# Harvard-AI-and-Robotics-Lab/FairFedMed

Measured on AMD Instinct MI355X. Metric: images/sec per client-round, ViT-B/16 FairLoRA r=8, bs=32 224^2, higher is better.
Workload: dtype bf16; 1 GPU; configs[1]: 1-client ViT-B/16 FairLoRA rank=8 G=3, bs=32 synthetic 224x224x3, fwd+bwd+SGD per step; global_batch=32, clients=1, trainable_elems=741952, loss_finite=1, launch=replay, rccl_ranks=1

## Files before the change

fairfedmed_amd/_lib.py:

```python
from __future__ import annotations

import ctypes as C
import os
from typing import Optional

import torch

_HERE = os.path.dirname(os.path.abspath(__file__))
LIB_PATH = os.environ.get("FFM_LIB_PATH") or os.path.join(_HERE, "csrc", "libffm_hip.so")

F32, BF16, F32_X3, F16 = 0, 1, 2, 3
F32_X3_W16 = 4
EPI_BIAS, EPI_LORA, EPI_LORA_KR, EPI_RESIDUAL, EPI_GELU, EPI_DGELU, EPI_RANKOP = 1, 2, 4, 8, 16, 32, 64
EPI_ROWSTATS, EPI_LNIN, EPI_LGRAD, EPI_BNBWD = 128, 256, 512, 1024
EPI_LNB_STAT, EPI_LNB_APPLY = 2048, 4096
EPI_GELU_ONLY = 8192
ABI_VERSION = 14

_vp, _i32, _i64, _f32 = C.c_void_p, C.c_int32, C.c_int64, C.c_float


class GemmArgs(C.Structure):
    _fields_ = [
        ("a", _vp), ("b", _vp), ("c", _vp),
# ... 64 lines not shown
    "ffm_bn_bwd": [_vp, _vp, _vp, _vp, _vp, _vp, _vp, _i32, _vp, _vp, _vp, _vp, _vp, _i32, _i32, _i32, _vp],
    "ffm_avgpool2": [_vp, _vp, _i32, _i32, _i32, _i32, _i32, _i32, _vp],
    "ffm_add": [_vp, _vp, _vp, C.c_int64, _i32, _vp],
    "ffm_relu_bwd": [_vp, _vp, _vp, C.c_int64, _i32, _vp],
    "ffm_attnpool_tokens": [_vp, _vp, _vp, _i32, _i32, _i32, _i32, _i32, _vp],
    "ffm_conv3x3_nhwc": [_vp, _vp, _vp, _i32, _i32, _i32, _i32, _i32, _i32, _vp, _vp, _i64, _vp, _i32, _vp],
    "ffm_conv3x3_nhwc_bnbwd": [_vp, _vp, _vp, _i32, _i32, _i32, _i32, _i32, _i32, _vp, _vp, _i64, _vp, _vp, _vp, _vp, _vp, _i32, _vp],
    "ffm_conv3x3_colstat_rows": [_i32, _i32, _i32, _i32, _i32, _i32, _i64, _i32],
    "ffm_eval_counts": [_vp, _vp, _vp, _i32, _i32, _vp, _vp],
    "ffm_eval_counts_ws_bytes": [_i32],
    "ffm_eval_counts_sorted": [_vp, _vp, _vp, _i32, _i32, _vp, _vp, _i64, _vp],
    "ffm_ot_head_fwd": [_vp] * 10 + [_i32] * 6 + [_f32, _f32, _i32, _f32, _i32, _vp],
    "ffm_ot_head_bwd": [_vp] * 8 + [_i32] * 6 + [_vp],
    "ffm_expand_u8": [_vp, _vp, _i32, _i32, _i32, _i32, _vp],
    "ffm_resize_u8": [_vp, _vp, _vp, _vp, _vp, _i32, _i32, _i32, _i32, _i32, _vp],
    "ffm_scale_check": [_vp, _f32, _i64, _vp, _vp],
    "ffm_attention_fwd": [_vp, _vp, _vp, _i32, _i32, _i32, _i32, _i32, _vp],
    "ffm_attention_bwd": [_vp, _vp, _vp, _vp, _vp, _vp, _i32, _i32, _i32, _i32, _i32, _vp],
    "ffm_attention_bwd_lnstat_ok": [_i32, _i32, _i32],
    "ffm_attention_bwd_lnstat": [_vp, _vp, _vp, _vp, _vp, _vp, _vp, _vp, _vp, _i32, _i32, _i32, _i32, _i32, _vp],
    "ffm_lora_down": [_vp, _i32, _vp, _i32, _vp, _vp, _i32, _i32, _i32, _i32, _i32, _f32, _f32, _vp, _vp, _vp, _vp,
                      _i32, _vp],
    "ffm_lora_down_blocks": [_i32, _i32, _i32, _i32],
    "ffm_lora_down_blocks_max": [_i32, _i32, _i32, _i32],
    "ffm_lora_grad_partial": [_vp, _i32, _vp, _i32, _i32, _i32, _vp, _i32, _vp],
    "ffm_lora_grad_partial_ln": [_vp, _i32, _vp, _vp, _vp, _vp, _vp, _i32, _i32, _i32, _vp, _i32, _vp],
    "ffm_lora_grad_splits": [_i32],
    "ffm_reduce_partials": [_vp, _i32, _i32, _vp, _i32, _i32, _i32, _vp],
    "ffm_reduce_partials_multi": [_vp, _i32, _i32, _vp],
    "ffm_head_fwd": [_vp, _vp, _vp, _vp, _vp, _vp, _i32, _i32, _i32, _i32, _i32, _vp],
    "ffm_ce_loss": [_vp, _vp, _vp, _vp, _vp, _vp, _vp, _i32, _i32, _i32, _vp],
    "ffm_ce_fair_loss": [_vp] * 10 + [_i32, _i32, _i32, _i32, _f32, _i32, _vp],
    "ffm_head_bwd": [_vp, _vp, _vp, _vp, _vp, _vp, _vp, _vp, _i32, _i32, _i32, _i32, _i32, _vp],
    "ffm_text_embed": [_vp, _vp, _vp, _i32, _vp, _vp, _i32, _i32, _i32, _i32, _i32, _vp],
    "ffm_text_tail_fwd": [_vp] * 10 + [_i32] * 4 + [_vp],
    "ffm_text_tail_bwd": [_vp] * 11 + [_i32] * 5 + [_vp],
    "ffm_text_ctx_grad": [_vp, _vp, _i32, _i32, _i32, _i32, _i32, _vp],
    "ffm_sgd_momentum": [_vp, _vp, _vp, _i64, _f32, _f32, _f32, _i32, _vp],
    "ffm_sgd_momentum_n": [_vp, _vp, _vp, _i64, _f32, _f32, _f32, _i32, _i32, _vp],
    "ffm_sgd_momentum_dev": [_vp, _vp, _vp, _i64, _vp, _i32, _vp, _vp],
    "ffm_loss_scale": [_vp, _i64, _vp, _vp],
    "ffm_unscale_check": [_vp, _i64, _vp, _vp],
    "ffm_sgd_momentum_gated": [_vp, _vp, _vp, _i64, _f32, _f32, _f32, _i32, _i32, _vp, _vp],
    "ffm_optim_state_rows": [_i32],
    "ffm_optim_step": [_vp, _vp, _vp, _i64, _i32, _vp, _i32, _vp, _vp],
    "ffm_optim_step_dev": [_vp, _vp, _vp, _i64, _i32, _vp, _i32, _vp, _vp],
    "ffm_scale_by": [_vp, _vp, _vp, _i64, _vp],
    "ffm_scale_acc": [_vp, _vp, _vp, _i64, _vp],
    "ffm_fedavg_finish": [_vp, _vp, _vp, _i64, _vp, _i32, _i32, _i32, _i32, _f32, _vp],
    "ffm_cast_f32_to": [_vp, _vp, _i64, _i32, _vp],
    "ffm_cast_to_f32": [_vp, _vp, _i64, _i32, _vp],
    "ffm_transpose_cast": [_vp, _vp, _i32, _i32, _i32, _vp],
}

_lib: Optional[C.CDLL] = None


def load() -> C.CDLL:
    global _lib
    if _lib is not None:
        return _lib
    if not os.path.exists(LIB_PATH):
        raise RuntimeError(
            f"{LIB_PATH} is missing: build it with `python -m fairfedmed_amd.build` "
            "(the FairLoRA engine has no fallback path)")
    lib = C.CDLL(LIB_PATH)
# ... 39 lines not shown
```

fairfedmed_amd/csrc/head.hip:

```cpp
#include "common.h"

namespace {

constexpr int HD_MAXV = 4;
constexpr int HD_MAXC = 8;

constexpr int HD_NW = 16;

template <typename T>
__global__ __launch_bounds__(64 * HD_NW) void head_fwd_kernel(const T* __restrict__ f, const float* __restrict__ tbar,
                                                       const float* __restrict__ logit_scale,
                                                       float* __restrict__ fbar, float* __restrict__ rnorm,
                                                       float* __restrict__ logits, int L, int D, int n_cls) {
    __shared__ float red[HD_NW / 2][4 * 64 * HD_MAXV];
    const int b = blockIdx.x, lane = threadIdx.x & 63, wave = threadIdx.x >> 6;
    const int nchunk = D >> 2;
    f32x4 acc[HD_MAXV];
#pragma unroll
    for (int i = 0; i < HD_MAXV; ++i) acc[i] = (f32x4){0.f, 0.f, 0.f, 0.f};
    for (int l = 1 + wave; l < L; l += HD_NW) {
        const T* fr = f + ((size_t)b * L + l) * D;
        f32x4 v[HD_MAXV];
        float ss = 0.f;
#pragma unroll
// ... 25 lines not shown
#pragma unroll
                for (int e = 0; e < 4; ++e) red[wave - HD_NW / 2][c * 4 + e] = acc[i][e];
            }
        }
    }
    __syncthreads();
    if (wave < HD_NW / 2) {
#pragma unroll
        for (int i = 0; i < HD_MAXV; ++i) {
            const int c = lane + 64 * i;
            if (c < nchunk) {
#pragma unroll
                for (int e = 0; e < 4; ++e) red[wave][c * 4 + e] += acc[i][e];
            }
        }
    }
    __syncthreads();
    const float inv = 1.0f / (float)(L - 1);
    for (int d = threadIdx.x; d < D; d += 64 * HD_NW) {
        float s = 0.f;
#pragma unroll
        for (int w = 0; w < HD_NW / 2; ++w) s += red[w][d];
        s *= inv;
        red[0][d] = s;
        fbar[(size_t)b * D + d] = s;
    }
    __syncthreads();
    const float scale = expf(logit_scale[0]);
    for (int c = wave; c < n_cls; c += HD_NW) {
        float s = 0.f;
        for (int d = lane; d < D; d += 64) s += red[0][d] * tbar[(size_t)c * D + d];
        s = wave_sum(s);
        if (lane == 0) logits[(size_t)b * n_cls + c] = scale * s;
    }
}

__global__ __launch_bounds__(256) void ce_loss_kernel(const float* __restrict__ logits_img,
                                                      const int64_t* __restrict__ label, float* __restrict__ logits,
                                                      float* __restrict__ prob, float* __restrict__ loss,
                                                      float* __restrict__ dlogits_img, int32_t* __restrict__ finite,
                                                      int nb, int S, int n_cls) {
    __shared__ float part[256];
    float my = 0.f;
    for (int b = threadIdx.x; b < nb; b += 256) {
        float lg[HD_MAXC];
        float mx = -INFINITY;
        for (int c = 0; c < n_cls; ++c) {
            float s = 0.f;
            for (int k = 0; k < S; ++k) s += logits_img[((size_t)b * S + k) * n_cls + c];
            lg[c] = s / (float)S;
            logits[(size_t)b * n_cls + c] = lg[c];
            mx = fmaxf(mx, lg[c]);
        }
        float se = 0.f;
        for (int c = 0; c < n_cls; ++c) se += expf(lg[c] - mx);
        const float lse = mx + logf(se);
        const int y = (int)label[b];
        my += lse - lg[y];
        for (int c = 0; c < n_cls; ++c) {
            const float pc = expf(lg[c] - lse);
            prob[(size_t)b * n_cls + c] = pc;
            const float dl = (pc - (c == y ? 1.f : 0.f)) / (float)nb / (float)S;
            for (int k = 0; k < S; ++k) dlogits_img[((size_t)b * S + k) * n_cls + c] = dl;
        }
    }
    part[threadIdx.x] = my;
// ... 152 lines not shown
            for (int i = 0; i < HD_MAXV; ++i) {
                const int c = lane + 64 * i;
                if (c < nchunk) Vec4<T>::store(dr + c * 4, (f32x4){0.f, 0.f, 0.f, 0.f});
            }
            continue;
        }
        const T* fr = f + ((size_t)b * L + l) * D;
        const float rn = rnorm[(size_t)b * L + l];
        f32x4 y[HD_MAXV];
        float dot = 0.f;
#pragma unroll
        for (int i = 0; i < HD_MAXV; ++i) {
            const int c = lane + 64 * i;
            if (c < nchunk) {
                const f32x4 v = Vec4<T>::load(fr + c * 4);
#pragma unroll
                for (int e = 0; e < 4; ++e) { y[i][e] = v[e] * rn; dot += y[i][e] * dyb[c * 4 + e]; }
            }
        }
        dot = wave_sum(dot);
#pragma unroll
        for (int i = 0; i < HD_MAXV; ++i) {
            const int c = lane + 64 * i;
            if (c < nchunk) {
                f32x4 o;
#pragma unroll
                for (int e = 0; e < 4; ++e) o[e] = (dyb[c * 4 + e] - y[i][e] * dot) * rn;
                Vec4<T>::store(dr + c * 4, o);
            }
        }
    }
}

__global__ __launch_bounds__(256) void head_dtbar_kernel(const float* __restrict__ fbar,
                                                         const float* __restrict__ logit_scale,
                                                         const float* __restrict__ dlogits, float* __restrict__ dtbar,
                                                         int B, int D, int n_cls) {
    const int i = blockIdx.x * blockDim.x + threadIdx.x;
    if (i >= n_cls * D) return;
    const int c = i / D, d = i % D;
    float s = 0.f;
    int b = 0;
    for (; b + 8 <= B; b += 8) {
        float dl[8], fb[8];
#pragma unroll
        for (int u = 0; u < 8; ++u) {
            dl[u] = dlogits[(size_t)(b + u) * n_cls + c];
            fb[u] = fbar[(size_t)(b + u) * D + d];
        }
#pragma unroll
        for (int u = 0; u < 8; ++u) s += dl[u] * fb[u];
    }
    for (; b < B; ++b) s += dlogits[(size_t)b * n_cls + c] * fbar[(size_t)b * D + d];
    dtbar[i] = s * expf(logit_scale[0]);
}

}

extern "C" int ffm_head_fwd(const void* f, const float* tbar, const float* logit_scale, float* fbar, float* rnorm,
                            float* logits_img, int B, int L, int D, int n_cls, int dtype, void* stream) {
    if (!f || !tbar || !logit_scale || !fbar || !rnorm || !logits_img) return FFM_EINVAL;
    if (B <= 0 || L <= 1 || D <= 0 || (D & 3) || D > 4 * 64 * HD_MAXV || n_cls <= 0 || n_cls > HD_MAXC) return FFM_EINVAL;
    hipStream_t s = (hipStream_t)stream;
    if (dtype == FFM_BF16)
        hipLaunchKernelGGL((head_fwd_kernel<bf16_t>), dim3(B), dim3(64 * HD_NW), 0, s, (const bf16_t*)f, tbar, logit_scale,
                           fbar, rnorm, logits_img, L, D, n_cls);
    else if (dtype == FFM_F32)
        hipLaunchKernelGGL((head_fwd_kernel<float>), dim3(B), dim3(64 * HD_NW), 0, s, (const float*)f, tbar, logit_scale,
                           fbar, rnorm, logits_img, L, D, n_cls);
    else
        return FFM_EINVAL;
    FFM_CHECK_LAUNCH();
    return FFM_OK;
}

extern "C" int ffm_ce_loss(const float* logits_img, const int64_t* label, float* logits, float* prob, float* loss,
                           float* dlogits_img, int32_t* finite_flag, int nb, int S, int n_cls, void* stream) {
    if (!logits_img || !label || !logits || !prob || !loss || !dlogits_img) return FFM_EINVAL;
    if (nb <= 0 || S <= 0 || n_cls <= 0 || n_cls > HD_MAXC) return FFM_EINVAL;
    hipLaunchKernelGGL(ce_loss_kernel, dim3(1), dim3(256), 0, (hipStream_t)stream, logits_img, label, logits, prob,
                       loss, dlogits_img, finite_flag, nb, S, n_cls);
    FFM_CHECK_LAUNCH();
    return FFM_OK;
}

extern "C" int ffm_ce_fair_loss(const float* logits_img, const int64_t* label, const int32_t* attr, float* logits,
                                float* prob, float* loss, float* terms, float* gstat, float* dlogits_img,
                                int32_t* finite_flag, int nb, int S, int n_cls, int G, float lambda, int with_grad,
                                void* stream) {
    if (!logits_img || !label || !attr || !logits || !prob || !loss || !terms || !dlogits_img) return FFM_EINVAL;
    if (nb <= 0 || S <= 0 || n_cls <= 0 || n_cls > HD_MAXC || G <= 0 || G > FFM_MAX_GROUPS) return FFM_EINVAL;
    hipLaunchKernelGGL(ce_fair_loss_kernel, dim3(1), dim3(256), 0, (hipStream_t)stream, logits_img, label, attr, logits,
                       prob, loss, terms, gstat, dlogits_img, finite_flag, nb, S, n_cls, G, lambda, with_grad ? 1 : 0);
    FFM_CHECK_LAUNCH();
    return FFM_OK;
}

extern "C" int ffm_head_bwd(const void* f, const float* tbar, const float* logit_scale, const float* fbar,
                            const float* rnorm, const float* dlogits_img, void* df, float* dtbar, int B, int L, int D,
                            int n_cls, int dtype, void* stream) {
    if (!f || !tbar || !logit_scale || !fbar || !rnorm || !dlogits_img || !df || !dtbar) return FFM_EINVAL;
    if (B <= 0 || L <= 1 || D <= 0 || (D & 3) || D > 4 * 64 * HD_MAXV || n_cls <= 0 || n_cls > HD_MAXC) return FFM_EINVAL;
    hipStream_t s = (hipStream_t)stream;
    if (dtype == FFM_BF16)
// ... 14 lines not shown
```

fairfedmed_amd/engine.py:

```python
from __future__ import annotations

import os
from dataclasses import dataclass
from typing import Dict, List, Optional, Tuple

import torch

from . import _lib as L
from ._lib import is16 as _is16
from . import ops
from .config import ModelCfg
from .data import NativeBatch
from .synth import manifest, trainable_keys

Tensor = torch.Tensor


def _round_up(x: int, m: int) -> int:
    return (x + m - 1) // m * m


class FlatParams:

    def __init__(self, cfg: ModelCfg, device):
# ... 370 lines not shown

    @grad_scale.setter
    def grad_scale(self, value: float) -> None:
        value = float(value)
        if not (value > 0.0) or value != value or value == float("inf"):
            raise ValueError(f"grad_scale must be a positive finite number, got {value!r}")
        if self.scale_state is None:
            if value != 1.0:
                raise ValueError("grad_scale exists in the IEEE-half mode only")
            return
        self.scale_state[:2].copy_(torch.tensor([value, 1.0 / value]))
        self.scale_state[5:6].fill_(max(value, float(self.scale_state[5])))

    def overflow_steps(self) -> int:
        return int(self.scale_state[4]) if self.scale_state is not None else 0

    def __init__(self, cfg: ModelCfg, state_dict: Dict[str, Tensor], dtype=torch.bfloat16, max_images: int = 32,
                 device: str = "cuda:0", max_infer_images: Optional[int] = None):
        if not torch.cuda.is_available():
            raise RuntimeError("FairLoRAEngine needs an MI355X GPU; there is no CPU path")
        from . import _lib
        _lib.load()
        if cfg.vision.head_dim != 64 or cfg.text.width // cfg.text.heads != 64:
            raise ValueError("attention kernels are built for head_dim 64 (all CLIP towers)")
        self.cfg, self.dtype, self.device = cfg, dtype, torch.device(device)
        self.max_images = max_images
        v, t = cfg.vision, cfg.text
        self.sw = Switches.from_env()
        self.fused_rank = 0 < cfg.lora.rank <= 16
        self.pack_plan = None
        self._pack_event = None
        self.pk_out: Dict[str, Tensor] = {}
        self.use_replay = True
        self.no_colstats, self.bn_bwd_fused = False, self.sw.bn_bwd_fused
        self.params = FlatParams(cfg, self.device)
        self.params.load(state_dict)
        self.n_text = cfg.n_prompts * cfg.n_cls
        self.txt_len = min(t.context_length, max(cfg.eot) + 1)
        assert self.txt_len >= 1 + cfg.n_ctx
        if not all(0 <= int(e) < self.txt_len for e in cfg.eot):
            raise ValueError(f"EOT positions {list(cfg.eot)} must lie inside the {self.txt_len} text rows that are kept "
                             f"(context_length {t.context_length})")
        self.txt = _Stack(t.width, t.heads, t.layers, self.txt_len, self.n_text, True, 0, torch.float32, self.device,
                          self.sw, x3=(_is16(dtype)))
        dev, f32 = self.device, torch.float32
        self._init_vision(max_images)
        self.load_frozen(state_dict)
        self._init_vision_late()
        self.feat = torch.zeros(max_images * v.tokens, v.out_dim, device=dev, dtype=dtype)
        self.dfeat = torch.zeros_like(self.feat)
        self.fbar = torch.zeros(max_images, v.out_dim, device=dev, dtype=f32)
        self.rnorm = torch.zeros(max_images * v.tokens, device=dev, dtype=f32)
        self.logits_img = torch.zeros(max_images, cfg.n_cls, device=dev, dtype=f32)
        self.dlogits_img = torch.zeros_like(self.logits_img)
        self.logits = torch.zeros(max_images, cfg.n_cls, device=dev, dtype=f32)
        self.prob = torch.zeros_like(self.logits)
        self.loss = torch.zeros(1, device=dev, dtype=f32)
        self.finite = torch.ones(1, device=dev, dtype=torch.int32)
        self.scale_state = None
        if dtype == torch.float16:
            s0 = self.sw.f16_grad_scale
            self.scale_state = torch.tensor([s0, 1.0 / s0, 1.0, 0.0, 0.0, s0, self.sw.f16_growth_interval, 1.0],
                                            device=dev, dtype=f32)
        self.dtbar = torch.zeros(cfg.n_cls, v.out_dim, device=dev, dtype=f32)
        self.attr_i32 = torch.zeros(max_images, device=dev, dtype=torch.int32)
        self.label_buf = torch.zeros(max_images, device=dev, dtype=torch.int64)
        self._counts_buf = None
        self._fair_lam, self._fair_grad, self._fair_step = 0.0, False, False
        self.loss_terms = torch.zeros(2, device=dev, dtype=f32)
        self.group_conf = torch.zeros(ops.MAX_GROUPS, 2, device=dev, dtype=f32)
        self.tbar_buf = torch.zeros(cfg.n_cls, v.out_dim, device=dev, dtype=f32)
        self.ot = cfg.ot if cfg.ot != "None" else None
        if self.ot:
            if self.ot not in ops.OT_MODES:
                raise NotImplementedError(cfg.ot)
            P, M, N = max_images * cfg.n_cls, v.tokens - 1, cfg.n_prompts
            self.dtn = torch.zeros(N * cfg.n_cls, v.out_dim, device=dev, dtype=f32)
            self.ot_sim = torch.zeros(P * M * N, device=dev, dtype=f32)
            self.ot_T = torch.zeros_like(self.ot_sim)
            self.ot_errs = torch.zeros(cfg.ot_max_iter * P, device=dev, dtype=f32)
            self.ot_istop = torch.zeros(1, device=dev, dtype=torch.int32)
            self.ot_tsum = torch.zeros(P, device=dev, dtype=f32)
            self.ot_dtn_part = torch.zeros(max_images * N * cfg.n_cls * v.out_dim, device=dev, dtype=f32)
        self.step_plans: Dict[tuple, list] = {}
# ... 502 lines not shown
        if train and self.sops.glob:
            self._glue(self.sops.prepare)
        ops.gemm_nt(ws.cols[:images * P], self.conv_w, ws.patch_out[:images * P], b_packed=self.pk_out.get("conv_w"))
        lb0 = bufs.layer(0, rows)
        ops.embed_lnpre(ws.patch_out[:images * P], self.cls, self.pos, self.lnpre[0], self.lnpre[1],
                        lb0.x, images, L, rowstat=lb0.rowp)
        if train:
            self._rank_operands_ready()
        out = self._stack_forward(self.vis, rows, images, a32, L * S, bufs)
        ops.layernorm_fwd(out, ws.hpost[:rows], self.lnpost[0], self.lnpost[1], ws.post_stats[0], ws.post_stats[1])
        ops.gemm_nt(ws.hpost[:rows], self.proj_t, ws.feat[:rows], b_packed=self.pk_out.get("proj_t"))
        if wait is not None:
            self._ev_wait(torch.cuda.current_stream(self.device), wait)
        self._head_forward(rows, images, L, ws)

    def _pack_rank_operands(self) -> None:
        if self.pack_plan is not None:
            self.pack_plan.run()

    def _rank_operands_ready(self) -> None:
        ev = self._pack_event
        if ev is None:
            self._pack_rank_operands()
        else:
            self._ev_wait(torch.cuda.current_stream(self.device), ev)

    def _head_forward(self, rows: int, images: int, L: int, ws=None) -> None:
        cfg = self.cfg
        ws = self if ws is None else ws
        if self.ot:
            ops.ot_head_fwd(ws.feat[:rows], self.tn_buf, self.logit_scale, ws.rnorm, ws.ot_sim, ws.ot_T, ws.ot_errs,
                            ws.ot_istop, ws.ot_tsum, ws.logits_img, images, L, cfg.n_cls, cfg.n_prompts, self.ot,
                            cfg.ot_eps, cfg.ot_thresh, cfg.ot_max_iter, cfg.ot_top_percent)
        else:
            ops.head_fwd(ws.feat[:rows], self.tbar_buf, self.logit_scale, ws.fbar, ws.rnorm, ws.logits_img,
                         images, L, cfg.n_cls)

    def _head_backward(self, rows: int, images: int, L: int) -> None:
        cfg = self.cfg
        if self.ot:
            P = cfg.n_prompts * cfg.n_cls
            ops.ot_head_bwd(self.feat[:rows], self.tn_buf, self.logit_scale, self.rnorm, self.ot_T, self.dlogits_img,
                            self.dfeat[:rows], self.ot_dtn_part, images, L, cfg.n_cls, cfg.n_prompts)
            ops.reduce_partials(self.ot_dtn_part, images, P * self.cfg.vision.out_dim, self.dtn.view(-1))
        else:
            ops.head_bwd(self.feat[:rows], self.tbar_buf, self.logit_scale, self.fbar, self.rnorm, self.dlogits_img,
                         self.dfeat[:rows], self.dtbar, images, L, cfg.n_cls)

    def _vision_backward(self, b: int, S: int, has_attr: bool) -> None:
        cfg, v = self.cfg, self.cfg.vision
        images, L = b * S, v.tokens
        rows = images * L
        a32 = self.attr_i32[:b] if has_attr else None
        ops.gemm_nt(self.dfeat[:rows], self.proj, self.vis.dh[:rows], b_packed=self.pk_out.get("proj"))
        gl = self.vis.rank > 0
        ops.layernorm_bwd(self.vis.dh[:rows], self.vis.x[v.layers][:rows], self.lnpost[0], self.post_stats[0],
                          self.post_stats[1], None, (self.vis.g_l[v.layers - 1] if gl else self.vis.g)[:rows])
        self._stack_backward(self.vis, rows, images, a32, L * S, self.is3d, grad_in_last=gl)
        if self.is3d:
            P = v.grid * v.grid
            ops.embed_lnpre_bwd(self.vis.g[:rows], self.patch_out[:images * P], self.pos, self.lnpre[0],
                                self.dpatch[:images * P], images, L)
            ops.gemm_nt(self.dpatch[:images * P], self.conv_w_t, self.dcols[:images * P])

    @torch.no_grad()
    def forward(self, image: Tensor, attr: Optional[Tensor] = None) -> Tensor:
        if self.sops.type != "FairLoRA":
            attr = None
        b, S = self._load_inputs(image, attr, None)
        self._text_forward(False)
        self._vision_forward(b, S, attr is not None)
        return self.logits_img[:b * S].view(b, S, -1).mean(1)

    def _infer_prepare(self) -> None:
        self._pack_rank_operands()
        if self.sops.glob:
            self.sops.prepare()
# ... 9 lines not shown
                self.prev, eng._in_session = eng._in_session, True
                return eng

            def __exit__(self, *a):
                eng._in_session = self.prev
                return False
        return _Session()

    @torch.no_grad()
    def infer(self, image: Tensor, attr: Optional[Tensor] = None) -> Tensor:
        if self.sops.type != "FairLoRA":
            attr = None
        ws = self.infer_ws
        b, S = self._load_inputs(image, attr, None, ws)
        if not self._in_session:
            self._infer_prepare()
        self._vision_forward(b, S, attr is not None, ws=ws)
        return ws.logits_img[:b * S].view(b, S, -1).mean(1)

    def _step_body(self, b: int, S: int, has_attr: bool) -> None:
        cfg, v = self.cfg, self.cfg.vision
        main = torch.cuda.current_stream(self.device)
        images, L = b * S, v.tokens
        rows = images * L
        a32 = self.attr_i32[:b] if has_attr else None
        self._ev_record(self.ev_start, main)
        self._ev_wait(self.side, self.ev_start)
        with self._on(self.side):
            self._pack_rank_operands()
            self._ev_record(self.ev_pack, self.side)
            self._text_forward(True, self.side)
        self._ev_record(self.ev_text_fwd, self.side)
        self._pack_event = self.ev_pack
        try:
            self._vision_forward(b, S, has_attr, wait=self.ev_text_fwd)
        finally:
            self._pack_event = None
        if self._fair_step:
            ops.ce_fair_loss(self.logits_img, self.label_buf, self.attr_i32, self.logits, self.prob, self.loss,
                             self.loss_terms, self.group_conf, self.dlogits_img, self.finite, b, S, cfg.n_cls,
                             self._fair_groups(), self._fair_lam, self._fair_grad)
        else:
            ops.ce_loss(self.logits_img, self.label_buf, self.logits, self.prob, self.loss, self.dlogits_img,
                        self.finite, b, S, cfg.n_cls)
        if self.scale_state is not None:
            ops.loss_scale(self.dlogits_img[:b * S], self.scale_state)
        self._head_backward(rows, images, L)
        self._ev_record(self.ev_head_bwd, main)
        self._ev_wait(self.side, self.ev_head_bwd)
        with self._on(self.side):
            if self._counts_buf is not None:
                ops.eval_counts(self.prob[:b], self.label_buf[:b], None, 0, method="pairs", out=self._counts_buf)
            self._text_backward(self.side)
        self._ev_record(self.ev_text_bwd, self.side)
        self._vision_backward(b, S, has_attr)
        self._ev_wait(main, self.ev_text_bwd)

    def forward_backward(self, image: Tensor, attr: Optional[Tensor], label: Tensor) -> Dict[str, Tensor]:
        fair = self._fair_lam != 0.0 and attr is not None
        loss_attr = attr if fair else None
        if self.sops.type != "FairLoRA":
            attr = None
        with torch.no_grad():
            b, S = self._load_inputs(image, attr if attr is not None else loss_attr, label)
            key = (b, S, attr is not None, torch.cuda.current_stream(self.device).cuda_stream) + (("fair",) if fair else ())
            self._fair_step = fair
            plan = self.step_plans.get(key) if self.use_replay else None
            if plan is not None:
                for f in plan:
                    f()
            elif self.use_replay:
                plan = []
                with ops.record(plan):
                    self._step_body(b, S, attr is not None)
                self.step_plans[key] = plan
            else:
                self._step_body(b, S, attr is not None)
            if self.is3d:
                images, P, D = b * S, self.cfg.vision.grid ** 2, self.cfg.dim_per_3d_slice
                ops.slice_bwd(self.dcols[:images * P], self._image, self.conv_out[:images], self.mnmx, self.mm_cnt,
                              self.dconv[:images], self.ab_part, self.gmm, self.wpart, D, self.cfg.vision.patch,
                              self.cfg.pixel_std)
                nw = 3 * D * 25 + 3
                off = self.params.offsets["proj_per_3d_slice.weight"][0]
                assert self.params.offsets["proj_per_3d_slice.bias"][0] == off + nw - 3
                nblk = ops.slice_wgrad_blocks(self.cfg.vision.image_size, self.cfg.vision.image_size)
                ops.reduce_partials(self.wpart, images * nblk, nw, self.params.grad[off:off + nw])
            if self.scale_state is not None:
                ops.unscale_check(self.params.grad, self.scale_state)
        out = {"loss": self.loss, "logits": self.logits[:b], "prob": self.prob[:b], "finite": self.finite}
        if self._counts_buf is not None:
            out["counts"] = self._counts_buf
        if fair:
            out["loss_terms"], out["group_conf"] = self.loss_terms, self.group_conf[:self._fair_groups()]
        return out

    @torch.no_grad()
    def sgd_step(self, lr: float, momentum: float, weight_decay: float, repeats: int = 1) -> None:
# ... 142 lines not shown
```

fairfedmed_amd/ops.py:

```python
from __future__ import annotations

import ctypes as C
from typing import Optional

import torch

from . import _lib as L

Tensor = torch.Tensor

_REC = None


class record:
    def __init__(self, plan: list):
        self.plan = plan

    def __enter__(self):
        global _REC
        self.prev, _REC = _REC, self.plan
        return self.plan

    def __exit__(self, *a):
        global _REC
# ... 698 lines not shown

def ce_loss(logits_img: Tensor, label: Tensor, logits: Tensor, prob: Tensor, loss: Tensor, dlogits_img: Tensor,
            finite: Optional[Tensor], nb: int, S: int, n_cls: int) -> None:
    _dev(logits_img, label, logits, prob, loss, dlogits_img, finite)
    assert label.dtype == torch.int64 and (finite is None or finite.dtype == torch.int32)
    _call("ffm_ce_loss", L.ptr(_f32(logits_img)), L.ptr(label), L.ptr(_f32(logits)), L.ptr(_f32(prob)),
                                 L.ptr(_f32(loss)), L.ptr(_f32(dlogits_img)), L.ptr(finite), nb, S, n_cls,
                                 L.stream_ptr())


def ce_fair_loss(logits_img: Tensor, label: Tensor, attr: Tensor, logits: Tensor, prob: Tensor, loss: Tensor,
                 terms: Tensor, gstat: Optional[Tensor], dlogits_img: Tensor, finite: Optional[Tensor], nb: int, S: int,
                 n_cls: int, G: int, lam: float, with_grad: bool = False) -> None:
    _dev(logits_img, label, attr, logits, prob, loss, terms, gstat, dlogits_img, finite)
    assert label.dtype == torch.int64 and attr.dtype == torch.int32 and (finite is None or finite.dtype == torch.int32)
    assert attr.is_contiguous() and attr.numel() >= nb and label.numel() >= nb and terms.numel() >= 2
    assert logits_img.numel() >= nb * S * n_cls and dlogits_img.numel() >= nb * S * n_cls
    assert logits.numel() >= nb * n_cls and prob.numel() >= nb * n_cls and (gstat is None or gstat.numel() >= 2 * G)
    _call("ffm_ce_fair_loss", L.ptr(_f32(logits_img)), L.ptr(label), L.ptr(attr), L.ptr(_f32(logits)), L.ptr(_f32(prob)),
          L.ptr(_f32(loss)), L.ptr(_f32(terms)), L.ptr(_f32(gstat)), L.ptr(_f32(dlogits_img)), L.ptr(finite), nb, S,
          n_cls, G, float(lam), int(bool(with_grad)), L.stream_ptr())


def head_bwd(f: Tensor, tbar: Tensor, logit_scale: Tensor, fbar: Tensor, rnorm: Tensor, dlogits_img: Tensor,
             df: Tensor, dtbar: Tensor, B: int, Ltok: int, n_cls: int) -> None:
    _dev(f, tbar, logit_scale, fbar, rnorm, dlogits_img, df, dtbar)
    D = f.shape[1]
    assert f.dtype == df.dtype and df.is_contiguous()
    _call("ffm_head_bwd", L.ptr(f), L.ptr(_f32(tbar)), L.ptr(_f32(logit_scale)), L.ptr(_f32(fbar)),
                                  L.ptr(_f32(rnorm)), L.ptr(_f32(dlogits_img)), L.ptr(df), L.ptr(_f32(dtbar)), B,
                                  Ltok, D, n_cls, L.dtype_code(f.dtype), L.stream_ptr())


def sgd_momentum(p: Tensor, g: Tensor, buf: Tensor, lr: float, momentum: float, weight_decay: float,
                 first_step: bool, repeats: int = 1) -> None:
    _dev(p, g, buf)
    if repeats == 1:
        _call("ffm_sgd_momentum", L.ptr(_f32(p)), L.ptr(_f32(g)), L.ptr(_f32(buf)), p.numel(), lr, momentum,
              weight_decay, int(first_step), L.stream_ptr())
    else:
        _call("ffm_sgd_momentum_n", L.ptr(_f32(p)), L.ptr(_f32(g)), L.ptr(_f32(buf)), p.numel(), lr, momentum,
              weight_decay, int(first_step), int(repeats), L.stream_ptr())


MAX_GROUPS = 8
SCALE_STATE = 8


def loss_scale(p: Tensor, state: Tensor) -> None:
    _dev(p, state)
    assert p.is_contiguous() and state.numel() == SCALE_STATE
    _call("ffm_loss_scale", L.ptr(_f32(p)), p.numel(), L.ptr(_f32(state)), L.stream_ptr())


def unscale_check(g: Tensor, state: Tensor) -> None:
    _dev(g, state)
    assert g.is_contiguous() and state.numel() == SCALE_STATE
    _call("ffm_unscale_check", L.ptr(_f32(g)), g.numel(), L.ptr(_f32(state)), L.stream_ptr())


def sgd_momentum_gated(p: Tensor, g: Tensor, buf: Tensor, lr: float, momentum: float, weight_decay: float,
                       first_step: bool, repeats: int, state: Tensor) -> None:
    _dev(p, g, buf, state)
    _call("ffm_sgd_momentum_gated", L.ptr(_f32(p)), L.ptr(_f32(g)), L.ptr(_f32(buf)), p.numel(), lr, momentum,
          weight_decay, int(first_step), int(repeats), L.ptr(_f32(state)), L.stream_ptr())

# ... 87 lines not shown
```

include/ffm_hip.h:

```cpp
#ifndef FFM_HIP_H
#define FFM_HIP_H

#include <stdint.h>

#ifdef __cplusplus
extern "C" {
#endif

#define FFM_F32 0
#define FFM_BF16 1
#define FFM_F32_X3 2
#define FFM_F16 3
#define FFM_F32_X3_W16 4

#define FFM_OK 0
#define FFM_EINVAL (-1)
#define FFM_EUNSUP (-2)

#define FFM_MAX_RANK 32
#define FFM_MAX_GROUPS 8

#define FFM_ABI_VERSION 14
int ffm_abi_version(void);

// ... 162 lines not shown
                          float* part, int dtype, void* stream);
int ffm_lora_grad_partial_ln(const void* x, int ldx, const float* v, const float* mean, const float* rstd,
                             const float* gamma, const float* beta, int M, int K, int r, float* part, int dtype,
                             void* stream);
int ffm_lora_grad_splits(int M);

int ffm_reduce_partials(const float* part, int nsplit, int n, float* out, int transpose_K,
                        int transpose_r, int accumulate, void* stream);

typedef struct ffm_reduce_desc {
    const float* part;
    float* out;
    int32_t nsplit, n, transpose_K, transpose_r;
} ffm_reduce_desc;
int ffm_reduce_partials_multi(const ffm_reduce_desc* descs_dev, int ndesc, int max_n, void* stream);

int ffm_head_fwd(const void* f, const float* tbar, const float* logit_scale, float* fbar,
                 float* rnorm, float* logits_img, int B, int L, int D, int n_cls, int dtype,
                 void* stream);

int ffm_ce_loss(const float* logits_img, const int64_t* label, float* logits, float* prob,
                float* loss, float* dlogits_img, int32_t* finite_flag, int nb, int S, int n_cls,
                void* stream);

int ffm_ce_fair_loss(const float* logits_img, const int64_t* label, const int32_t* attr,
                     float* logits, float* prob, float* loss, float* terms, float* gstat,
                     float* dlogits_img, int32_t* finite_flag, int nb, int S, int n_cls, int G,
                     float lambda, int with_grad, void* stream);

int ffm_head_bwd(const void* f, const float* tbar, const float* logit_scale, const float* fbar,
                 const float* rnorm, const float* dlogits_img, void* df, float* dtbar, int B,
                 int L, int D, int n_cls, int dtype, void* stream);

int ffm_text_embed(const float* prefix, const float* ctx, const float* suffix, int suffix_rows, const float* pos, float* x,
                   int n_prompts, int n_cls, int n_ctx, int TL, int w, void* stream);
int ffm_text_tail_fwd(const float* x, const int32_t* eot_row, const float* lnw, const float* lnb, const float* proj,
                      float* tf, float* tn, float* rnorm, float* stats, float* tbar, int n_prompts, int n_cls, int w,
                      int D, void* stream);
int ffm_text_tail_bwd(const float* x, const int32_t* eot_row, const float* lnw, const float* proj, const float* tn,
                      const float* rnorm, const float* stats, const float* dtbar, const float* dtn, float* dy, float* g,
                      int n_prompts, int n_cls, int TL, int w, int D, void* stream);
int ffm_text_ctx_grad(const float* g, float* dctx, int n_prompts, int n_cls, int n_ctx, int TL, int w, void* stream);

int ffm_expand_u8(const uint8_t* src, float* dst, int B, int C1, int HW, int rep, void* stream);

#define FFM_RESIZE_MAX_TAPS 32
int ffm_resize_u8(const uint8_t* pix, const int32_t* geom, const int32_t* tab_start, const float* tab_w, float* dst,
                  int B, int C1, int rep, int R, int T, void* stream);

#define FFM_EVAL_SLOTS 10
int ffm_eval_counts(const float* prob, const int64_t* label, const int64_t* attr, int N, int G, uint64_t* out,
                    void* stream);
int64_t ffm_eval_counts_ws_bytes(int N);
int ffm_eval_counts_sorted(const float* prob, const int64_t* label, const int64_t* attr, int N, int G, uint64_t* out,
                           void* workspace, int64_t workspace_bytes, void* stream);

int ffm_ot_head_fwd(const void* f, const float* tn, const float* logit_scale, float* rnorm, float* sim, float* T,
                    float* errs, int32_t* istop, float* tsum, float* logits_img, int B, int L, int D, int n_cls,
                    int N, int mode, float eps, float thresh, int max_iter, float top_percent, int dtype, void* stream);
int ffm_ot_head_bwd(const void* f, const float* tn, const float* logit_scale, const float* rnorm, const float* T,
                    const float* dlogits_img, void* df, float* dtn_part, int B, int L, int D, int n_cls, int N,
                    int dtype, void* stream);

int ffm_sgd_momentum(float* p, const float* g, float* buf, int64_t n, float lr, float momentum,
                     float weight_decay, int first_step, void* stream);

// ... 48 lines not shown
```

Before: 7203 images/sec.

## Split head forward across waves and fuse CE loss into head backward

Replaces the single-block-per-image head forward with a multi-block kernel that writes per-wave partial pooled features. A new head backward kernel reduces those partials itself, computes logits and the cross-entropy gradient inline, and spreads the dfeat writes over four blocks per image. The full CE loss and dtbar computation move to the side stream, off the main critical path. This path is limited to non-fair, S==1, non-OT, unscaled steps and adds an fpart buffer plus redundant per-block reductions.

```diff
diff --git a/fairfedmed_amd/_lib.py b/fairfedmed_amd/_lib.py
--- a/fairfedmed_amd/_lib.py
+++ b/fairfedmed_amd/_lib.py
@@ -120,6 +120,9 @@
     "ffm_ce_loss": [_vp, _vp, _vp, _vp, _vp, _vp, _vp, _i32, _i32, _i32, _vp],
     "ffm_ce_fair_loss": [_vp] * 10 + [_i32, _i32, _i32, _i32, _f32, _i32, _vp],
     "ffm_head_bwd": [_vp, _vp, _vp, _vp, _vp, _vp, _vp, _vp, _i32, _i32, _i32, _i32, _i32, _vp],
+    "ffm_head_fwd_split": [_vp, _vp, _vp, _i32, _i32, _i32, _i32, _vp],
+    "ffm_head_bwd_self": [_vp] * 10 + [_i32, _i32, _i32, _i32, _i32, _vp],
+    "ffm_head_dtbar": [_vp, _vp, _vp, _vp, _i32, _i32, _i32, _vp],
     "ffm_text_embed": [_vp, _vp, _vp, _i32, _vp, _vp, _i32, _i32, _i32, _i32, _i32, _vp],
     "ffm_text_tail_fwd": [_vp] * 10 + [_i32] * 4 + [_vp],
     "ffm_text_tail_bwd": [_vp] * 11 + [_i32] * 5 + [_vp],
diff --git a/fairfedmed_amd/csrc/head.hip b/fairfedmed_amd/csrc/head.hip
--- a/fairfedmed_amd/csrc/head.hip
+++ b/fairfedmed_amd/csrc/head.hip
@@ -81,6 +81,65 @@
         for (int d = lane; d < D; d += 64) s += red[0][d] * tbar[(size_t)c * D + d];
         s = wave_sum(s);
         if (lane == 0) logits[(size_t)b * n_cls + c] = scale * s;
+    }
+}
+
+constexpr int HD_PF = 4;
+
+__device__ __forceinline__ float sum_sq4(const f32x4 v) {
+#pragma clang fp contract(off)
+    return v[0] * v[0] + v[1] * v[1] + v[2] * v[2] + v[3] * v[3];
+}
+
+template <typename T>
+__global__ __launch_bounds__(64) void head_fwd_split_kernel(const T* __restrict__ f, float* __restrict__ fpart,
+                                                            float* __restrict__ rnorm, int L, int D) {
+    const int b = blockIdx.x, wave = blockIdx.y, lane = threadIdx.x;
+    const int nchunk = D >> 2;
+    f32x4 acc[HD_MAXV];
+#pragma unroll
+    for (int i = 0; i < HD_MAXV; ++i) acc[i] = (f32x4){0.f, 0.f, 0.f, 0.f};
+    for (int l0 = 1 + wave; l0 < L; l0 += HD_NW * HD_PF) {
+        f32x4 v[HD_PF][HD_MAXV];
+#pragma unroll
+        for (int u = 0; u < HD_PF; ++u) {
+            const int l = l0 + u * HD_NW;
+            const T* fr = f + ((size_t)b * L + (l < L ? l : l0)) * D;
+#pragma unroll
+            for (int i = 0; i < HD_MAXV; ++i) {
+                const int c = lane + 64 * i;
+                if (c < nchunk) v[u][i] = Vec4<T>::load(fr + c * 4);
+            }
+        }
+#pragma unroll
+        for (int u = 0; u < HD_PF; ++u) {
+            const int l = l0 + u * HD_NW;
+            if (l >= L) break;
+            float ss = 0.f;
+#pragma unroll
+            for (int i = 0; i < HD_MAXV; ++i) {
+                const int c = lane + 64 * i;
+                if (c < nchunk) ss += sum_sq4(v[u][i]);
+            }
+            const float nrm = sqrtf(wave_sum(ss));
+            const float rn = 1.0f / fmaxf(nrm, 1e-12f);
+            if (lane == 0) rnorm[(size_t)b * L + l] = rn;
+#pragma unroll
+            for (int i = 0; i < HD_MAXV; ++i) {
+                const int c = lane + 64 * i;
+                if (c < nchunk) {
+#pragma unroll
+                    for (int e = 0; e < 4; ++e) acc[i][e] += v[u][i][e] * rn;
+                }
+            }
+        }
+    }
+    if (wave == 0 && lane == 0) rnorm[(size_t)b * L] = 0.f;
+    float* fp = fpart + ((size_t)b * HD_NW + wave) * D;
+#pragma unroll
+    for (int i = 0; i < HD_MAXV; ++i) {
+        const int c = lane + 64 * i;
+        if (c < nchunk) *reinterpret_cast<f32x4*>(fp + c * 4) = acc[i];
     }
 }
 
@@ -299,6 +358,124 @@
     }
 }
 
+template <typename T>
+__global__ __launch_bounds__(64 * HD_NW) void head_bwd_self_kernel(const T* __restrict__ f, const float* __restrict__ tbar,
+                                                            const float* __restrict__ logit_scale,
+                                                            const float* __restrict__ fpart,
+                                                            const float* __restrict__ rnorm,
+                                                            const int64_t* __restrict__ label, T* __restrict__ df,
+                                                            float* __restrict__ fbar, float* __restrict__ logits_img,
+                                                            float* __restrict__ dlogits_img, int nb, int L, int D,
+                                                            int n_cls) {
+    __shared__ float dyb[4 * 64 * HD_MAXV];
+    __shared__ float sfb[4 * 64 * HD_MAXV];
+    __shared__ float slog[HD_MAXC];
+    const int b = blockIdx.x, lane = threadIdx.x & 63, wave = threadIdx.x >> 6;
+    const int nchunk = D >> 2;
+    const bool keeper = blockIdx.y == 0;
+    const float* fp = fpart + (size_t)b * HD_NW * D;
+    const float inv = 1.0f / (float)(L - 1);
+    for (int d = threadIdx.x; d < D; d += 64 * HD_NW) {
+        float r[HD_NW / 2];
+#pragma unroll
+        for (int w = 0; w < HD_NW / 2; ++w) {
+            r[w] = fp[(size_t)(w + HD_NW / 2) * D + d];
+            r[w] += fp[(size_t)w * D + d];
+        }
+        float s = 0.f;
+#pragma unroll
+        for (int w = 0; w < HD_NW / 2; ++w) s += r[w];
+        s *= inv;
+        sfb[d] = s;
+        if (keeper) fbar[(size_t)b * D + d] = s;
+    }
+    __syncthreads();
+    const float escale = expf(logit_scale[0]);
+    for (int c = wave; c < n_cls; c += HD_NW) {
+        float s = 0.f;
+        for (int d = lane; d < D; d += 64) s += sfb[d] * tbar[(size_t)c * D + d];
+        s = wave_sum(s);
+        if (lane == 0) slog[c] = escale * s;
+    }
+    __syncthreads();
+    float dl[HD_MAXC];
+    {
+        float lg[HD_MAXC];
+        float mx = -INFINITY;
+#pragma unroll
+        for (int c = 0; c < HD_MAXC; ++c) {
+            if (c < n_cls) {
+                float s = 0.f;
+                s += slog[c];
+                lg[c] = s / 1.0f;
+                mx = fmaxf(mx, lg[c]);
+            }
+        }
+        float se = 0.f;
+#pragma unroll
+        for (int c = 0; c < HD_MAXC; ++c)
+            if (c < n_cls) se += expf(lg[c] - mx);
+        const float lse = mx + logf(se);
+        const int y = (int)label[b];
+#pragma unroll
+        for (int c = 0; c < HD_MAXC; ++c) {
+            dl[c] = 0.f;
+            if (c < n_cls) {
+                const float pc = expf(lg[c] - lse);
+                dl[c] = (pc - (c == y ? 1.f : 0.f)) / (float)nb / 1.0f;
+                if (keeper && threadIdx.x == 0) {
+                    logits_img[(size_t)b * n_cls + c] = slog[c];
+                    dlogits_img[(size_t)b * n_cls + c] = dl[c];
+                }
+            }
+        }
+    }
+    const float scale = escale / (float)(L - 1);
+    for (int d = threadIdx.x; d < D; d += 64 * HD_NW) {
+        float s = 0.f;
+#pragma unroll
+        for (int c = 0; c < HD_MAXC; ++c)
+            if (c < n_cls) s += dl[c] * tbar[(size_t)c * D + d];
+        dyb[d] = s * scale;
+    }
+    __syncthreads();
+    for (int l = blockIdx.y * HD_NW + wave; l < L; l += HD_NW * gridDim.y) {
+        T* dr = df + ((size_t)b * L + l) * D;
+        if (l == 0) {
+#pragma unroll
+            for (int i = 0; i < HD_MAXV; ++i) {
+                const int c = lane + 64 * i;
+                if (c < nchunk) Vec4<T>::store(dr + c * 4, (f32x4){0.f, 0.f, 0.f, 0.f});
+            }
+            continue;
+        }
+        const T* fr = f + ((size_t)b * L + l) * D;
+        const float rn = rnorm[(size_t)b * L + l];
+        f32x4 y[HD_MAXV];
+        float dot = 0.f;
+#pragma unroll
+        for (int i = 0; i < HD_MAXV; ++i) {
+            const int c = lane + 64 * i;
+            if (c < nchunk) {
+                const f32x4 v = Vec4<T>::load(fr + c * 4);
+#pragma unroll
+                for (int e = 0; e < 4; ++e) { y[i][e] = v[e] * rn; dot += y[i][e] * dyb[c * 4 + e]; }
+            }
+        }
+        dot = wave_sum(dot);
+#pragma unroll
+        for (int i = 0; i < HD_MAXV; ++i) {
+            const int c = lane + 64 * i;
+            if (c < nchunk) {
+                f32x4 o;
+#pragma unroll
+                for (int e = 0; e < 4; ++e) o[e] = (dyb[c * 4 + e] - y[i][e] * dot) * rn;
+                Vec4<T>::store(dr + c * 4, o);
+            }
+        }
+    }
+}
+
 __global__ __launch_bounds__(256) void head_dtbar_kernel(const float* __restrict__ fbar,
                                                          const float* __restrict__ logit_scale,
                                                          const float* __restrict__ dlogits, float* __restrict__ dtbar,
@@ -337,6 +514,53 @@
                            fbar, rnorm, logits_img, L, D, n_cls);
     else
         return FFM_EINVAL;
+    FFM_CHECK_LAUNCH();
+    return FFM_OK;
+}
+
+extern "C" int ffm_head_fwd_split(const void* f, float* fpart, float* rnorm, int B, int L, int D, int dtype,
+                                  void* stream) {
+    if (!f || !fpart || !rnorm) return FFM_EINVAL;
+    if (B <= 0 || L <= 1 || D <= 0 || (D & 3) || D > 4 * 64 * HD_MAXV) return FFM_EINVAL;
+    if (((uintptr_t)fpart & 15)) return FFM_EINVAL;
+    hipStream_t s = (hipStream_t)stream;
+    if (dtype == FFM_BF16)
+        hipLaunchKernelGGL((head_fwd_split_kernel<bf16_t>), dim3(B, HD_NW), dim3(64), 0, s, (const bf16_t*)f, fpart, rnorm,
+                           L, D);
+    else if (dtype == FFM_F32)
+        hipLaunchKernelGGL((head_fwd_split_kernel<float>), dim3(B, HD_NW), dim3(64), 0, s, (const float*)f, fpart, rnorm, L,
+                           D);
+    else
+        return FFM_EINVAL;
+    FFM_CHECK_LAUNCH();
+    return FFM_OK;
+}
+
+extern "C" int ffm_head_bwd_self(const void* f, const float* tbar, const float* logit_scale, const float* fpart,
+                                 const float* rnorm, const int64_t* label, void* df, float* fbar, float* logits_img,
+                                 float* dlogits_img, int B, int L, int D, int n_cls, int dtype, void* stream) {
+    if (!f || !tbar || !logit_scale || !fpart || !rnorm || !label || !df || !fbar || !logits_img || !dlogits_img)
+        return FFM_EINVAL;
+    if (B <= 0 || L <= 1 || D <= 0 || (D & 3) || D > 4 * 64 * HD_MAXV || n_cls <= 0 || n_cls > HD_MAXC) return FFM_EINVAL;
+    hipStream_t s = (hipStream_t)stream;
+    if (dtype == FFM_BF16)
+        hipLaunchKernelGGL((head_bwd_self_kernel<bf16_t>), dim3(B, 4), dim3(64 * HD_NW), 0, s, (const bf16_t*)f, tbar,
+                           logit_scale, fpart, rnorm, label, (bf16_t*)df, fbar, logits_img, dlogits_img, B, L, D, n_cls);
+    else if (dtype == FFM_F32)
+        hipLaunchKernelGGL((head_bwd_self_kernel<float>), dim3(B, 4), dim3(64 * HD_NW), 0, s, (const float*)f, tbar,
+                           logit_scale, fpart, rnorm, label, (float*)df, fbar, logits_img, dlogits_img, B, L, D, n_cls);
+    else
+        return FFM_EINVAL;
+    FFM_CHECK_LAUNCH();
+    return FFM_OK;
+}
+
+extern "C" int ffm_head_dtbar(const float* fbar, const float* logit_scale, const float* dlogits_img, float* dtbar, int B,
+                              int D, int n_cls, void* stream) {
+    if (!fbar || !logit_scale || !dlogits_img || !dtbar) return FFM_EINVAL;
+    if (B <= 0 || D <= 0 || n_cls <= 0 || n_cls > HD_MAXC) return FFM_EINVAL;
+    hipLaunchKernelGGL(head_dtbar_kernel, dim3((n_cls * D + 255) / 256), dim3(256), 0, (hipStream_t)stream, fbar,
+                       logit_scale, dlogits_img, dtbar, B, D, n_cls);
     FFM_CHECK_LAUNCH();
     return FFM_OK;
 }
diff --git a/fairfedmed_amd/engine.py b/fairfedmed_amd/engine.py
--- a/fairfedmed_amd/engine.py
+++ b/fairfedmed_amd/engine.py
@@ -426,6 +426,8 @@
         self._pack_event = None
         self.pk_out: Dict[str, Tensor] = {}
         self.use_replay = True
+        self.split_neck = True
+        self._neck_split = False
         self.no_colstats, self.bn_bwd_fused = False, self.sw.bn_bwd_fused
         self.params = FlatParams(cfg, self.device)
         self.params.load(state_dict)
@@ -444,6 +446,7 @@
         self.feat = torch.zeros(max_images * v.tokens, v.out_dim, device=dev, dtype=dtype)
         self.dfeat = torch.zeros_like(self.feat)
         self.fbar = torch.zeros(max_images, v.out_dim, device=dev, dtype=f32)
+        self.fpart = torch.zeros(max_images, ops.HEAD_WAVES, v.out_dim, device=dev, dtype=f32)
         self.rnorm = torch.zeros(max_images * v.tokens, device=dev, dtype=f32)
         self.logits_img = torch.zeros(max_images, cfg.n_cls, device=dev, dtype=f32)
         self.dlogits_img = torch.zeros_like(self.logits_img)
@@ -1012,6 +1015,8 @@
             ops.ot_head_fwd(ws.feat[:rows], self.tn_buf, self.logit_scale, ws.rnorm, ws.ot_sim, ws.ot_T, ws.ot_errs,
                             ws.ot_istop, ws.ot_tsum, ws.logits_img, images, L, cfg.n_cls, cfg.n_prompts, self.ot,
                             cfg.ot_eps, cfg.ot_thresh, cfg.ot_max_iter, cfg.ot_top_percent)
+        elif self._neck_split and ws is self:
+            ops.head_fwd_split(ws.feat[:rows], self.fpart, ws.rnorm, images, L)
         else:
             ops.head_fwd(ws.feat[:rows], self.tbar_buf, self.logit_scale, ws.fbar, ws.rnorm, ws.logits_img,
                          images, L, cfg.n_cls)
@@ -1023,6 +1028,9 @@
             ops.ot_head_bwd(self.feat[:rows], self.tn_buf, self.logit_scale, self.rnorm, self.ot_T, self.dlogits_img,
                             self.dfeat[:rows], self.ot_dtn_part, images, L, cfg.n_cls, cfg.n_prompts)
             ops.reduce_partials(self.ot_dtn_part, images, P * self.cfg.vision.out_dim, self.dtn.view(-1))
+        elif self._neck_split:
+            ops.head_bwd_self(self.feat[:rows], self.tbar_buf, self.logit_scale, self.fpart, self.rnorm, self.label_buf,
+                              self.dfeat[:rows], self.fbar, self.logits_img, self.dlogits_img, images, L, cfg.n_cls)
         else:
             ops.head_bwd(self.feat[:rows], self.tbar_buf, self.logit_scale, self.fbar, self.rnorm, self.dlogits_img,
                          self.dfeat[:rows], self.dtbar, images, L, cfg.n_cls)
@@ -1098,23 +1106,30 @@
             self._text_forward(True, self.side)
         self._ev_record(self.ev_text_fwd, self.side)
         self._pack_event = self.ev_pack
+        split = self._neck_split = (self.split_neck and not self._fair_step and S == 1 and not self.ot
+                                    and self.scale_state is None)
         try:
             self._vision_forward(b, S, has_attr, wait=self.ev_text_fwd)
+            if self._fair_step:
+                ops.ce_fair_loss(self.logits_img, self.label_buf, self.attr_i32, self.logits, self.prob, self.loss,
+                                 self.loss_terms, self.group_conf, self.dlogits_img, self.finite, b, S, cfg.n_cls,
+                                 self._fair_groups(), self._fair_lam, self._fair_grad)
+            elif not split:
+                ops.ce_loss(self.logits_img, self.label_buf, self.logits, self.prob, self.loss, self.dlogits_img,
+                            self.finite, b, S, cfg.n_cls)
+            if self.scale_state is not None:
+                ops.loss_scale(self.dlogits_img[:b * S], self.scale_state)
+            self._head_backward(rows, images, L)
         finally:
             self._pack_event = None
-        if self._fair_step:
-            ops.ce_fair_loss(self.logits_img, self.label_buf, self.attr_i32, self.logits, self.prob, self.loss,
-                             self.loss_terms, self.group_conf, self.dlogits_img, self.finite, b, S, cfg.n_cls,
-                             self._fair_groups(), self._fair_lam, self._fair_grad)
-        else:
-            ops.ce_loss(self.logits_img, self.label_buf, self.logits, self.prob, self.loss, self.dlogits_img,
-                        self.finite, b, S, cfg.n_cls)
-        if self.scale_state is not None:
-            ops.loss_scale(self.dlogits_img[:b * S], self.scale_state)
-        self._head_backward(rows, images, L)
+            self._neck_split = False
         self._ev_record(self.ev_head_bwd, main)
         self._ev_wait(self.side, self.ev_head_bwd)
         with self._on(self.side):
+            if split:
+                ops.ce_loss(self.logits_img, self.label_buf, self.logits, self.prob, self.loss, self.dlogits_img,
+                            self.finite, b, S, cfg.n_cls)
+                ops.head_dtbar(self.fbar, self.logit_scale, self.dlogits_img, self.dtbar, images, cfg.n_cls)
             if self._counts_buf is not None:
                 ops.eval_counts(self.prob[:b], self.label_buf[:b], None, 0, method="pairs", out=self._counts_buf)
             self._text_backward(self.side)
@@ -1130,6 +1145,8 @@
         with torch.no_grad():
             b, S = self._load_inputs(image, attr if attr is not None else loss_attr, label)
             key = (b, S, attr is not None, torch.cuda.current_stream(self.device).cuda_stream) + (("fair",) if fair else ())
+            if not self.split_neck:
+                key += ("classic",)
             self._fair_step = fair
             plan = self.step_plans.get(key) if self.use_replay else None
             if plan is not None:
diff --git a/fairfedmed_amd/ops.py b/fairfedmed_amd/ops.py
--- a/fairfedmed_amd/ops.py
+++ b/fairfedmed_amd/ops.py
@@ -754,6 +754,37 @@
                                   Ltok, D, n_cls, L.dtype_code(f.dtype), L.stream_ptr())
 
 
+HEAD_WAVES = 16
+
+
+def head_fwd_split(f: Tensor, fpart: Tensor, rnorm: Tensor, B: int, Ltok: int) -> None:
+    _dev(f, fpart, rnorm)
+    D = f.shape[1]
+    assert f.is_contiguous() and f.shape[0] >= B * Ltok and rnorm.numel() >= B * Ltok and fpart.numel() >= B * HEAD_WAVES * D
+    _call("ffm_head_fwd_split", L.ptr(f), L.ptr(_f32(fpart)), L.ptr(_f32(rnorm)), B, Ltok, D, L.dtype_code(f.dtype),
+          L.stream_ptr())
+
+
+def head_bwd_self(f: Tensor, tbar: Tensor, logit_scale: Tensor, fpart: Tensor, rnorm: Tensor, label: Tensor, df: Tensor,
+                  fbar: Tensor, logits_img: Tensor, dlogits_img: Tensor, B: int, Ltok: int, n_cls: int) -> None:
+    _dev(f, tbar, logit_scale, fpart, rnorm, label, df, fbar, logits_img, dlogits_img)
+    D = f.shape[1]
+    assert f.dtype == df.dtype and f.is_contiguous() and df.is_contiguous() and label.dtype == torch.int64
+    assert label.numel() >= B and fpart.numel() >= B * HEAD_WAVES * D and fbar.numel() >= B * D
+    assert logits_img.numel() >= B * n_cls and dlogits_img.numel() >= B * n_cls and df.shape[0] >= B * Ltok
+    _call("ffm_head_bwd_self", L.ptr(f), L.ptr(_f32(tbar)), L.ptr(_f32(logit_scale)), L.ptr(_f32(fpart)), L.ptr(_f32(rnorm)),
+          L.ptr(label), L.ptr(df), L.ptr(_f32(fbar)), L.ptr(_f32(logits_img)), L.ptr(_f32(dlogits_img)), B, Ltok, D, n_cls,
+          L.dtype_code(f.dtype), L.stream_ptr())
+
+
+def head_dtbar(fbar: Tensor, logit_scale: Tensor, dlogits_img: Tensor, dtbar: Tensor, B: int, n_cls: int) -> None:
+    _dev(fbar, logit_scale, dlogits_img, dtbar)
+    D = fbar.shape[1]
+    assert fbar.shape[0] >= B and dlogits_img.numel() >= B * n_cls and dtbar.numel() >= n_cls * D
+    _call("ffm_head_dtbar", L.ptr(_f32(fbar)), L.ptr(_f32(logit_scale)), L.ptr(_f32(dlogits_img)), L.ptr(_f32(dtbar)), B, D,
+          n_cls, L.stream_ptr())
+
+
 def sgd_momentum(p: Tensor, g: Tensor, buf: Tensor, lr: float, momentum: float, weight_decay: float,
                  first_step: bool, repeats: int = 1) -> None:
     _dev(p, g, buf)
diff --git a/include/ffm_hip.h b/include/ffm_hip.h
--- a/include/ffm_hip.h
+++ b/include/ffm_hip.h
@@ -218,6 +218,15 @@
                  const float* rnorm, const float* dlogits_img, void* df, float* dtbar, int B,
                  int L, int D, int n_cls, int dtype, void* stream);
 
+int ffm_head_fwd_split(const void* f, float* fpart, float* rnorm, int B, int L, int D, int dtype,
+                       void* stream);
+int ffm_head_bwd_self(const void* f, const float* tbar, const float* logit_scale,
+                      const float* fpart, const float* rnorm, const int64_t* label, void* df,
+                      float* fbar, float* logits_img, float* dlogits_img, int B, int L, int D,
+                      int n_cls, int dtype, void* stream);
+int ffm_head_dtbar(const float* fbar, const float* logit_scale, const float* dlogits_img,
+                   float* dtbar, int B, int D, int n_cls, void* stream);
+
 int ffm_text_embed(const float* prefix, const float* ctx, const float* suffix, int suffix_rows, const float* pos, float* x,
                    int n_prompts, int n_cls, int n_ctx, int TL, int w, void* stream);
 int ffm_text_tail_fwd(const float* x, const int32_t* eot_row, const float* lnw, const float* lnb, const float* proj,
```

Result: no change. 7241 images/sec, median of 6 (+0.5%).
